# VivianDLi/CryoVIT

Hardware: AMD Instinct MI355X
Metric: tomogram voxels/sec (DINO feats + 3D seg fwd) (higher is better)
Workload: dtype bf16; 1 GPU; one 128x512x512 uint8 tomogram per step per GPU (configs[3]'s seeds 100..131, rank r takes 100 + r*steps + i): fused resize + DINOv2 ViT-g/14-reg (40 layers, N=1029 tokens/slice) -> fp16 dino_features [1536,128,32,32] + CryoVIT head [1,1536,128,32,32] -> probs [128,512,512] + masked Dice; synthetic weights; slice_batch=128, streams=1, parallelism=tomogram-sharded x1, no collectives

## Files before the change

cryovit_amd/check_asm.py:

```python

from __future__ import annotations

import re
import subprocess
import sys
import tempfile
from pathlib import Path

from cryovit_amd.build import ARCH, CSRC, FILE_FLAGS, FLAGS, INCLUDE, hipcc_path

EXPECTED_STORES = {"EpiSwiGLU": 8, "EpiBF16": 16, "EpiResidT": 32, "EpiResidHL": 33, "EpiVT": 16}


def compile_asm(src: Path) -> str:
    with tempfile.TemporaryDirectory() as td:
        out = Path(td) / (src.stem + ".s")
        flags = [f for f in FLAGS if f != "-fPIC"]
        cmd = [hipcc_path(), *flags, *FILE_FLAGS.get(src.name, []), "-I", str(INCLUDE), "-S", "--cuda-device-only", "-o", str(out), str(src)]
        r = subprocess.run(cmd, capture_output=True, text=True)
        if r.returncode != 0:
            raise RuntimeError(f"hipcc -S failed on {src.name}:\n{r.stderr}")
        return out.read_text()


def check_gemm256p(asm: str) -> list[str]:
    bodies = {m.group(1): m.group(2) for m in re.finditer(r"^(_ZN3cvx15k_gemm256p_[nm]reg\w+):.*?\n(.*?)s_endpgm", asm, re.S | re.M)}
    assert bodies, "no k_gemm256p kernels in the assembly"
    report = []
    for m in re.finditer(r"\.amdhsa_kernel (_ZN3cvx15k_gemm256p_[nm]reg\w+)(.*?)\.end_amdhsa_kernel", asm, re.S):
        name, desc = m.group(1), m.group(2)
        body = bodies[name]
        scratch = int(re.search(r"\.amdhsa_private_segment_fixed_size (\d+)", desc).group(1))
        vgpr = int(re.search(r"\.amdhsa_next_free_vgpr (\d+)", desc).group(1))
        assert scratch == 0 and "scratch_" not in body, f"{name}: spills to scratch ({scratch} B): uncounted vmcnt entries"
        assert vgpr <= 256, f"{name}: {vgpr} VGPRs"
        dma = re.findall(r"global_load_lds_dwordx4 (.*)", body)
        assert dma and all(re.fullmatch(r"v\d+, s\[\d+:\d+\]", d.strip()) for d in dma), f"{name}: LDS-DMA not in saddr form: {set(dma)}"
        stores = len(re.findall(r"global_store_", body))
        full = re.search(r"ELb1E(Lb[01]E)?EEv", name) is not None
        kind = next(k for k in EXPECTED_STORES if k in name)
        if full:
            assert stores == EXPECTED_STORES[kind], f"{name}: {stores} store instructions, the waits assume {EXPECTED_STORES[kind]}"
            assert all(s.startswith("global_store_dwordx4") for s in re.findall(r"global_store_\w+", body)), name
        report.append(f"{name[24:70]:48s} vgpr {vgpr:3d} stores {stores:2d} dma {len(dma):2d} {'FULL' if full else 'edge'}")
    return report


def check_dma_users(asm: str, fname: str) -> list[str]:
    report, inside, kernel, n_dma = [], False, None, {}
    for ln in asm.splitlines():
        t = ln.strip()
        m = re.match(r"^(_Z\w+):", ln)
        if m:
            kernel = m.group(1)
        if "#ASMSTART" in t:
            inside = True
        elif "#ASMEND" in t:
            inside = False
        elif t and not t.startswith((";", ".", "//")):
            if "global_load_lds" in t:
                n_dma[kernel] = n_dma.get(kernel, 0) + 1
            if not inside:
                assert "global_load_lds" not in t, f"{fname}:{kernel}: compiler-generated LDS-DMA: {t}"
                assert not re.search(r"\bm0\b", t), f"{fname}:{kernel}: M0 touched outside inline asm: {t}"
    for m in re.finditer(r"\.amdhsa_kernel (\w+)(.*?)\.end_amdhsa_kernel", asm, re.S):
        name, desc = m.group(1), m.group(2)
        if name not in n_dma:
            continue
        scratch = int(re.search(r"\.amdhsa_private_segment_fixed_size (\d+)", desc).group(1))
        vgpr = int(re.search(r"\.amdhsa_next_free_vgpr (\d+)", desc).group(1))
        assert scratch == 0, f"{fname}:{name}: {scratch} B of scratch in a kernel with counted vector-memory waits"
        report.append(f"{fname:16s} {name[:60]:60s} vgpr {vgpr:3d} dma {n_dma[name]:3d}")
    return report


DMA_SOURCES = ("attention.hip", "conv_halo.hip")


def main() -> None:
    gemm_asm = compile_asm(CSRC / "gemm.hip")
    for line in check_gemm256p(gemm_asm):
        print(line)
    for line in check_dma_users(gemm_asm, "gemm.hip"):
        print(line)
    for f in DMA_SOURCES:
        for line in check_dma_users(compile_asm(CSRC / f), f):
            print(line)
    print("ok")


if __name__ == "__main__":
    assert ARCH == "gfx950"
    main()
```

cryovit_amd/csrc/attention.hip:

```cpp
#include "common.h"
#include "../../include/cryovit_hip.h"
#include "host_util.h"
#include <atomic>
#include <string.h>

namespace cvx {

constexpr int ATT_THREADS = 256;
constexpr int KV_TILE = 64;
constexpr int ATT_TILE_BYTES = 64 * 128;
constexpr int ATT_XCD_REMAP = 1;
constexpr int ATT_PRIO_QK = 2;
constexpr int ATT_PRIO_PV = 4;
constexpr int ATT_FULL_LAST_TILE = 8;

__device__ __forceinline__ int pi_row(int r) { return (r & 0x13) | ((r & 4) << 1) | ((r & 8) >> 1); }

enum class Softmax { RunningMax, TileMax, ProbSum };
struct AttnCfg {
    int waves = 4;
    int nbuf = 2;
    Softmax softmax = Softmax::RunningMax;
    bool legacy = false;
    bool no_exp = false, no_sync = false, no_dma = false;
};
constexpr AttnCfg attn_cfg(int variant) {
    AttnCfg c;
    switch (variant) {
        case 1: c.legacy = true; break;
        case 3: c.nbuf = 3; break;
        case 6: c.softmax = Softmax::TileMax; break;
        case 7: c.softmax = Softmax::ProbSum; break;
        case 8: c.softmax = Softmax::ProbSum; c.waves = 8; c.nbuf = 3; break;
        case 9: c.softmax = Softmax::ProbSum; c.waves = 8; break;
        case 10: c.no_exp = true; break;
        case 11: c.no_sync = c.no_dma = true; break;
        case 12: c.no_sync = true; break;
        case 13: c.no_dma = true; break;
    }
    return c;
}

struct BlockCoord { int qb, slice, head; };
__device__ __forceinline__ BlockCoord block_coord(int flags, int nqb, int heads) {
    int qb, pair;
    if (flags & ATT_XCD_REMAP) {
        const int xcd = blockIdx.x & 7, w = blockIdx.x >> 3;
        pair = (w / nqb) * 8 + xcd;
        qb = w % nqb;
    } else {
        pair = blockIdx.x / nqb;
        qb = blockIdx.x % nqb;
    }
    return {qb, pair / heads, pair % heads};
}

__device__ __forceinline__ float row_max(const f32x16 (&s)[2]) {
    float m = s[0][0];
#pragma unroll
    for (int i = 1; i < 16; ++i) m = fmaxf(m, s[0][i]);
#pragma unroll
    for (int i = 0; i < 16; ++i) m = fmaxf(m, s[1][i]);
    return fmaxf(m, __shfl_xor(m, 32, 64));
}

__device__ __forceinline__ void exp2_sum(f32x16 (&s)[2], float& psum) {
    psum = 0.f;
#pragma unroll
    for (int t = 0; t < 2; ++t)
#pragma unroll
        for (int i = 0; i < 16; ++i) {
            const float p = __builtin_amdgcn_exp2f(s[t][i]);
            s[t][i] = p;
            psum += p;
        }
}

typedef short v4s_t __attribute__((ext_vector_type(4)));
typedef short v8s_t __attribute__((ext_vector_type(8)));
template <int VARIANT, bool VROW = false>
__global__ __launch_bounds__(attn_cfg(VARIANT).waves * 64) void k_attention(const uint16_t* __restrict__ qk, long ldqk,
                                                                            const uint16_t* __restrict__ vt, uint16_t* __restrict__ out,
                                                                            long ldo, int heads, int ntok, int ntp, int kp, int C, int nqb,
                                                                            int flags) {
    constexpr AttnCfg cfg = attn_cfg(VARIANT);
    constexpr int NW = cfg.waves, NBUF = cfg.nbuf;
    constexpr int NT = NW * 64, QB = NW * 32;
    constexpr int PPT = 512 / NT;
    constexpr bool AUG = cfg.softmax != Softmax::RunningMax, PSUM_TRIGGER = cfg.softmax == Softmax::ProbSum;
    constexpr bool LEGACY = cfg.legacy, ABL_NOEXP = cfg.no_exp, ABL_NOSYNC = cfg.no_sync, ABL_NODMA = cfg.no_dma;
    __shared__ __attribute__((aligned(16))) char smem[NBUF * 2 * ATT_TILE_BYTES];
    const int tid = threadIdx.x, lane = tid & 63;
    const int wave = __builtin_amdgcn_readfirstlane(tid >> 6);
    const bool prio_qk = (flags & ATT_PRIO_QK) != 0, prio_pv = (flags & ATT_PRIO_PV) != 0;
    const BlockCoord bc = block_coord(flags, nqb, heads);
    const int qb = bc.qb, slice = bc.slice, head = bc.head;
    const long row0 = (long)slice * ntp;
    const uint16_t* Qp = qk + row0 * ldqk + head * 64;
    const uint16_t* Kp = Qp + C;
    const uint16_t* Vp = VROW ? Kp + C : vt + ((long)(slice * heads + head) * 64) * kp;
    const long vpitch = VROW ? ldqk : (long)kp;

    const int r = lane & 31, h = lane >> 5;
    const int q0 = qb * QB + wave * 32;
    const int qrow = min(q0 + r, ntp - 1);
    const bool wave_idle = !LEGACY && q0 >= ntok;

    bf16x8 qf[4];
    {
        const uint16_t* qsrc = Qp + (long)qrow * ldqk + 8 * h;
#pragma unroll
        for (int ks = 0; ks < 4; ++ks) asm volatile("global_load_dwordx4 %0, %1, off" : "=v"(qf[ks]) : "v"(qsrc + 16 * ks) : "memory");
    }
    constexpr float DEFER = 3.0f;
    bf16x8 kaug, qaug;
    [[maybe_unused]] float m_used = 0.f;
    if constexpr (AUG) {
#pragma unroll
        for (int e = 0; e < 8; ++e) { kaug[e] = (__bf16)0.f; qaug[e] = (__bf16)0.f; }
        if (h == 0) kaug[0] = (__bf16)1.0f;
    }

    uint32_t koffs[2], voffs[2];
#pragma unroll
    for (int jj = 0; jj < 2; ++jj) {
        const int c = (jj < PPT ? jj : 0) * NT + tid;
        const int srow = c >> 3, schunk = ((c & 7) ^ ((srow >> 1) & 7)) << 3;
        koffs[jj] = (uint32_t)(srow * ldqk + schunk) * 2u;
        voffs[jj] = (uint32_t)(srow * vpitch + schunk) * 2u;
    }
    const bool lone = AUG && qb * QB + 32 >= ntok;
    if (lone && wave != 0) return;
    auto issue = [&](int j, int buf) {
        const uint32_t kt = lds_addr(smem) + buf * 2 * ATT_TILE_BYTES + wave * 1024;
        const long kv0 = (long)j * KV_TILE;
        if constexpr (PPT == 2) {
            glds16_saddr2<NT * 16>(Kp + kv0 * ldqk, koffs[0], koffs[1], kt);
            glds16_saddr2<NT * 16>(Vp + (VROW ? kv0 * ldqk : kv0), voffs[0], voffs[1], kt + ATT_TILE_BYTES);
        } else {
            glds16_saddr(Kp + kv0 * ldqk, koffs[0], kt);
            glds16_saddr(Vp + (VROW ? kv0 * ldqk : kv0), voffs[0], kt + ATT_TILE_BYTES);
        }
        if (lone) {
            uint32_t k0 = koffs[0], k1 = koffs[1], v0 = voffs[0], v1 = voffs[1];
            asm volatile("" : "+v"(k0), "+v"(k1), "+v"(v0), "+v"(v1));
#pragma unroll 1
            for (int w2 = 1; w2 < NW; ++w2) {
                const uint32_t fl = (w2 & 1) ? 64u : 0u;
                const uint32_t dk = (uint32_t)(w2 * 16) * (uint32_t)ldqk, dv = (uint32_t)(w2 * 16) * (uint32_t)vpitch;
                if constexpr (PPT == 2) {
                    glds16_saddr2<NT * 16>(Kp + kv0 * ldqk, (k0 + dk) ^ fl, (k1 + dk) ^ fl, kt + w2 * 1024);
                    glds16_saddr2<NT * 16>(Vp + (VROW ? kv0 * ldqk : kv0), (v0 + dv) ^ fl, (v1 + dv) ^ fl, kt + ATT_TILE_BYTES + w2 * 1024);
                } else {
                    glds16_saddr(Kp + kv0 * ldqk, (k0 + dk) ^ fl, kt + w2 * 1024);
                    glds16_saddr(Vp + (VROW ? kv0 * ldqk : kv0), (v0 + dv) ^ fl, kt + ATT_TILE_BYTES + w2 * 1024);
                }
            }
        }
    };

    const int krow = pi_row(r);
    const int koff = krow * 128, ksw = (krow >> 1) & 7;
    const int voff = r * 128, vsw = (r >> 1) & 7;
    [[maybe_unused]] uint32_t vtr[2][2];
    if constexpr (VROW) {
        const int li = lane & 15, dgrp = (lane >> 4) & 1;
#pragma unroll
        for (int dt = 0; dt < 2; ++dt)
#pragma unroll
            for (int j = 0; j < 2; ++j) {
                const int row = 8 * h + 4 * j + (li >> 2);
                const int chunk = (4 * dt + 2 * dgrp + ((li & 3) >> 1)) ^ ((row >> 1) & 7);
                vtr[dt][j] = (uint32_t)(row * 128 + (chunk << 4) + (li & 1) * 8);
            }
    }

    f32x16 o[2];
#pragma unroll
    for (int i = 0; i < 16; ++i) { o[0][i] = 0.f; o[1][i] = 0.f; }
    float m_run = -INFINITY, l_run = 0.f;

    const int nkv = (ntok + KV_TILE - 1) / KV_TILE;
    issue(0, 0);
    if (NBUF == 3 && nkv > 1) issue(1, 1);
    asm volatile("s_waitcnt vmcnt(0)" : "+v"(qf[0]), "+v"(qf[1]), "+v"(qf[2]), "+v"(qf[3])::"memory");
    int buf = 0;
    const char* kt = smem;
    [[maybe_unused]] bool redo = false;
    for (int j = 0; j < nkv; ++j) {
        if (!PSUM_TRIGGER || !redo) {
        if (!ABL_NOSYNC || j == 0) {
            if (NBUF == 3 && j + 1 < nkv) {
                if (lone) asm volatile("s_waitcnt vmcnt(%0)" ::"n"(2 * PPT * NW) : "memory");
                else asm volatile("s_waitcnt vmcnt(%0)" ::"n"(2 * PPT) : "memory");
            } else asm volatile("s_waitcnt vmcnt(0)" ::: "memory");
            __builtin_amdgcn_s_barrier();
        }
        if (NBUF == 3) {
            if (j + 2 < nkv) issue(j + 2, buf == 0 ? 2 : buf - 1);
        } else if (!ABL_NODMA && j + 1 < nkv) {
            issue(ABL_NOSYNC ? 0 : j + 1, ABL_NOSYNC ? 1 : (buf ^ 1));
        }
        kt = smem + (ABL_NOSYNC || ABL_NODMA ? 0 : buf) * 2 * ATT_TILE_BYTES;
        buf = NBUF == 3 ? (buf == 2 ? 0 : buf + 1) : (buf ^ 1);
        }
        [[maybe_unused]] const bool anchor = j == 0 || redo;
        redo = false;
        const char* vtile = kt + ATT_TILE_BYTES;
        if (wave_idle) continue;

        f32x16 s[2];
        const int kv0 = j * KV_TILE;
        const bool half_tile = !(flags & ATT_FULL_LAST_TILE) && kv0 + 32 >= ntok;
        auto compute_s = [&]() {
#pragma unroll
            for (int i = 0; i < 16; ++i) { s[0][i] = 0.f; s[1][i] = 0.f; }
            if (prio_qk) __builtin_amdgcn_s_setprio(1);
#pragma unroll
            for (int t = 0; t < 2; ++t) {
                if (t == 1 && half_tile) break;
                if constexpr (AUG) s[t] = __builtin_amdgcn_mfma_f32_32x32x16_bf16(kaug, qaug, s[t], 0, 0, 0);
#pragma unroll
                for (int ks = 0; ks < 4; ++ks) {
                    const bf16x8 kf = *(const bf16x8*)(kt + t * 4096 + koff + (((2 * ks + h) ^ ksw) << 4));
                    s[t] = __builtin_amdgcn_mfma_f32_32x32x16_bf16(kf, qf[ks], s[t], 0, 0, 0);
                }
            }
            if (prio_qk) __builtin_amdgcn_s_setprio(0);
            if (kv0 + KV_TILE > ntok) {
#pragma unroll
                for (int t = 0; t < 2; ++t)
#pragma unroll
                    for (int i = 0; i < 16; ++i) {
                        const int rho = (i & 3) + 8 * (i >> 2) + 4 * h;
                        if (kv0 + 32 * t + pi_row(rho) >= ntok) s[t][i] = -INFINITY;
                    }
            }
        };
        compute_s();

        if constexpr (PSUM_TRIGGER) {
            float psum;
            if (anchor) {
                const float mloc = row_max(s);
                const float m_new = (float)(__bf16)(m_used + (j == 0 ? mloc : fmaxf(mloc, 0.f)));
                const float delta = m_new - m_used;
                m_used = m_new;
                if (h == 0) qaug[0] = (__bf16)(-m_new);
                const float alpha = j == 0 ? 1.0f : __builtin_amdgcn_exp2f(-delta);
                l_run *= alpha;
#pragma unroll
                for (int i = 0; i < 16; ++i) { o[0][i] *= alpha; o[1][i] *= alpha; s[0][i] -= delta; s[1][i] -= delta; }
            }
            exp2_sum(s, psum);
            if (!anchor && __builtin_amdgcn_ballot_w64(!(psum <= 16777216.0f)) != 0) {
                redo = true;
                --j;
                continue;
            }
            l_run += psum;
        } else if constexpr (AUG) {
            const float mloc = row_max(s);
            if (j == 0 || __builtin_amdgcn_ballot_w64(mloc > DEFER) != 0) {
                const float m_new = (float)(__bf16)(m_used + (j == 0 ? mloc : fmaxf(mloc, 0.f)));
                const float delta = m_new - m_used;
                m_used = m_new;
                if (h == 0) qaug[0] = (__bf16)(-m_new);
                const float alpha = j == 0 ? 1.0f : __builtin_amdgcn_exp2f(-delta);
                l_run *= alpha;
#pragma unroll
                for (int i = 0; i < 16; ++i) { o[0][i] *= alpha; o[1][i] *= alpha; s[0][i] -= delta; s[1][i] -= delta; }
            }
            float psum;
            exp2_sum(s, psum);
            l_run += psum;
        } else {
            const float m_new = fmaxf(m_run, row_max(s));
            const float alpha = __builtin_amdgcn_exp2f(m_run - m_new);
            m_run = m_new;
            float psum = 0.f;
#pragma unroll
            for (int t = 0; t < 2; ++t)
#pragma unroll
                for (int i = 0; i < 16; ++i) {
                    const float p = ABL_NOEXP ? (s[t][i] - m_new) * 0.001f : __builtin_amdgcn_exp2f(s[t][i] - m_new);
                    s[t][i] = p;
                    psum += p;
                }
            l_run = fmaf(l_run, alpha, psum);
            if (LEGACY || __builtin_amdgcn_ballot_w64(alpha != 1.0f) != 0) {
#pragma unroll
                for (int i = 0; i < 16; ++i) { o[0][i] *= alpha; o[1][i] *= alpha; }
            }
        }

        if (prio_pv) __builtin_amdgcn_s_setprio(1);
#pragma unroll
        for (int t = 0; t < 2; ++t) {
            if (t == 1 && half_tile) break;
#pragma unroll
            for (int sk = 0; sk < 2; ++sk) {
                bf16x8 pf;
#pragma unroll
                for (int e = 0; e < 8; ++e) pf[e] = (__bf16)s[t][8 * sk + e];
#pragma unroll
                for (int dt = 0; dt < 2; ++dt) {
                    bf16x8 vf;
                    if constexpr (VROW) {
                        typedef __attribute__((address_space(3))) v4s_t* lds_v4;
                        const char* vb = vtile + (32 * t + 16 * sk) * 128;
                        const v4s_t a = __builtin_amdgcn_ds_read_tr16_b64_v4i16((lds_v4)(vb + vtr[dt][0]));
                        const v4s_t b = __builtin_amdgcn_ds_read_tr16_b64_v4i16((lds_v4)(vb + vtr[dt][1]));
                        vf = __builtin_bit_cast(bf16x8, v8s_t{a[0], a[1], a[2], a[3], b[0], b[1], b[2], b[3]});
                    } else {
                        vf = *(const bf16x8*)(vtile + dt * 4096 + voff + (((4 * t + 2 * sk + h) ^ vsw) << 4));
                    }
                    o[dt] = __builtin_amdgcn_mfma_f32_32x32x16_bf16(vf, pf, o[dt], 0, 0, 0);
                }
            }
        }
        if (prio_pv) __builtin_amdgcn_s_setprio(0);
    }

    const float l_tot = l_run + __shfl_xor(l_run, 32, 64);
    const float inv = 1.0f / l_tot;
    if (q0 + r < ntok) {
        uint16_t* orow = out + (row0 + q0 + r) * ldo + head * 64;
#pragma unroll
        for (int dt = 0; dt < 2; ++dt)
#pragma unroll
            for (int g = 0; g < 4; ++g) {
                uint2 w;
                w.x = pack2bf(o[dt][4 * g + 0] * inv, o[dt][4 * g + 1] * inv);
                w.y = pack2bf(o[dt][4 * g + 2] * inv, o[dt][4 * g + 3] * inv);
                *(uint2*)(orow + 32 * dt + 8 * g + 4 * h) = w;
            }
    }
}

#ifdef CVX_ABLATION
template <int NW>
__global__ __launch_bounds__(NW * 64) void k_attention64(const uint16_t* __restrict__ qk, long ldqk, const uint16_t* __restrict__ vt,
                                                         uint16_t* __restrict__ out, long ldo, int heads, int ntok, int ntp, int kp,
                                                         int C, int nqb, int flags) {
    constexpr int NT = NW * 64;
    __shared__ __attribute__((aligned(16))) char smem[2 * 2 * ATT_TILE_BYTES];
    const int tid = threadIdx.x, lane = tid & 63;
    const int wave = __builtin_amdgcn_readfirstlane(tid >> 6);
    const BlockCoord bc = block_coord(flags, nqb, heads);
    const int qb = bc.qb, slice = bc.slice, head = bc.head;
    const long row0 = (long)slice * ntp;
    const uint16_t* Qp = qk + row0 * ldqk + head * 64;
    const uint16_t* Kp = Qp + C;
    const uint16_t* Vp = vt + ((long)(slice * heads + head) * 64) * kp;
    const int r = lane & 31, h = lane >> 5;
    const int q0 = qb * NT + wave * 64;

    bf16x8 qf[2][4];
#pragma unroll
    for (int g = 0; g < 2; ++g) {
        const int qrow = min(q0 + 32 * g + r, ntp - 1);
#pragma unroll
        for (int ks = 0; ks < 4; ++ks) qf[g][ks] = *(const bf16x8*)(Qp + (long)qrow * ldqk + 16 * ks + 8 * h);
    }
    constexpr int NP = (512 + NT - 1) / NT;
    uint32_t koffs[NP], voffs[NP];
#pragma unroll
    for (int jj = 0; jj < NP; ++jj) {
        const int c = jj * NT + tid;
        const int srow = (c >> 3) & 63, schunk = ((c & 7) ^ ((srow >> 1) & 7)) << 3;
        koffs[jj] = (uint32_t)(srow * ldqk + schunk) * 2u;
        voffs[jj] = (uint32_t)(srow * kp + schunk) * 2u;
    }
    auto issue = [&](int j, int buf) {
        const uint32_t kt = lds_addr(smem) + buf * 2 * ATT_TILE_BYTES;
        const long kv0 = (long)j * KV_TILE;
#pragma unroll
        for (int jj = 0; jj < NP; ++jj) {
            if (jj * NT + wave * 64 >= 512) break;
            glds16_saddr(Kp + kv0 * ldqk, koffs[jj], kt + (jj * NT + wave * 64) * 16);
            glds16_saddr(Vp + kv0, voffs[jj], kt + ATT_TILE_BYTES + (jj * NT + wave * 64) * 16);
        }
    };
    const int krow = pi_row(r);
    const int koff = krow * 128, ksw = (krow >> 1) & 7;
    const int voff = r * 128, vsw = (r >> 1) & 7;

    f32x16 o[2][2];
#pragma unroll
    for (int g = 0; g < 2; ++g)
#pragma unroll
        for (int i = 0; i < 16; ++i) { o[g][0][i] = 0.f; o[g][1][i] = 0.f; }
    float m_run[2] = {-INFINITY, -INFINITY}, l_run[2] = {0.f, 0.f};
    const int nkv = (ntok + KV_TILE - 1) / KV_TILE;

    issue(0, 0);
    for (int j = 0; j < nkv; ++j) {
        asm volatile("s_waitcnt vmcnt(0)" ::: "memory");
        __syncthreads();
        if (j + 1 < nkv) issue(j + 1, (j + 1) & 1);
        const char* kt = smem + (j & 1) * 2 * ATT_TILE_BYTES;
        const char* vtile = kt + ATT_TILE_BYTES;

        f32x16 s[2][2];
#pragma unroll
        for (int g = 0; g < 2; ++g)
#pragma unroll
            for (int i = 0; i < 16; ++i) { s[g][0][i] = 0.f; s[g][1][i] = 0.f; }
#pragma unroll
        for (int t = 0; t < 2; ++t)
#pragma unroll
            for (int ks = 0; ks < 4; ++ks) {
                const bf16x8 kf = *(const bf16x8*)(kt + t * 4096 + koff + (((2 * ks + h) ^ ksw) << 4));
                s[0][t] = __builtin_amdgcn_mfma_f32_32x32x16_bf16(kf, qf[0][ks], s[0][t], 0, 0, 0);
                s[1][t] = __builtin_amdgcn_mfma_f32_32x32x16_bf16(kf, qf[1][ks], s[1][t], 0, 0, 0);
            }
        const int kv0 = j * KV_TILE;
        if (kv0 + KV_TILE > ntok) {
#pragma unroll
            for (int g = 0; g < 2; ++g)
#pragma unroll
                for (int t = 0; t < 2; ++t)
#pragma unroll
                    for (int i = 0; i < 16; ++i) {
                        const int rho = (i & 3) + 8 * (i >> 2) + 4 * h;
                        if (kv0 + 32 * t + pi_row(rho) >= ntok) s[g][t][i] = -INFINITY;
                    }
        }
#pragma unroll
        for (int g = 0; g < 2; ++g) {
            const float m_new = fmaxf(m_run[g], row_max(s[g]));
            const float alpha = __builtin_amdgcn_exp2f(m_run[g] - m_new);
            m_run[g] = m_new;
            float psum = 0.f;
#pragma unroll
            for (int t = 0; t < 2; ++t)
#pragma unroll
                for (int i = 0; i < 16; ++i) {
                    const float p = __builtin_amdgcn_exp2f(s[g][t][i] - m_new);
                    s[g][t][i] = p;
                    psum += p;
                }
            l_run[g] = fmaf(l_run[g], alpha, psum);
            if (__builtin_amdgcn_ballot_w64(alpha != 1.0f) != 0) {
#pragma unroll
                for (int i = 0; i < 16; ++i) { o[g][0][i] *= alpha; o[g][1][i] *= alpha; }
            }
        }
#pragma unroll
        for (int t = 0; t < 2; ++t)
#pragma unroll
            for (int sk = 0; sk < 2; ++sk) {
                bf16x8 pf[2];
#pragma unroll
                for (int g = 0; g < 2; ++g)
#pragma unroll
                    for (int e = 0; e < 8; ++e) pf[g][e] = (__bf16)s[g][t][8 * sk + e];
#pragma unroll
                for (int dt = 0; dt < 2; ++dt) {
                    const bf16x8 vf = *(const bf16x8*)(vtile + dt * 4096 + voff + (((4 * t + 2 * sk + h) ^ vsw) << 4));
                    o[0][dt] = __builtin_amdgcn_mfma_f32_32x32x16_bf16(vf, pf[0], o[0][dt], 0, 0, 0);
                    o[1][dt] = __builtin_amdgcn_mfma_f32_32x32x16_bf16(vf, pf[1], o[1][dt], 0, 0, 0);
                }
            }
    }
#pragma unroll
    for (int g = 0; g < 2; ++g) {
        const float l_tot = l_run[g] + __shfl_xor(l_run[g], 32, 64);
        const float inv = 1.0f / l_tot;
        const int q = q0 + 32 * g + r;
        if (q < ntok) {
            uint16_t* orow = out + (row0 + q) * ldo + head * 64;
#pragma unroll
            for (int dt = 0; dt < 2; ++dt)
#pragma unroll
                for (int gg = 0; gg < 4; ++gg) {
                    uint2 w;
                    w.x = pack2bf(o[g][dt][4 * gg + 0] * inv, o[g][dt][4 * gg + 1] * inv);
                    w.y = pack2bf(o[g][dt][4 * gg + 2] * inv, o[g][dt][4 * gg + 3] * inv);
                    *(uint2*)(orow + 32 * dt + 8 * gg + 4 * h) = w;
                }
        }
    }
}

#endif

}

using namespace cvx;

typedef void (*attn_kernel_t)(const uint16_t*, long, const uint16_t*, uint16_t*, long, int, int, int, int, int, int, int);
struct AttnVariant {
    int id;
    attn_kernel_t kernel;
    int threads, rows;
    bool needs_ld64;
};
template <int V>
static AttnVariant attn_row() {
    constexpr AttnCfg c = attn_cfg(V);
    return {V, k_attention<V, false>, c.waves * 64, c.waves * 32, c.softmax != Softmax::RunningMax};
}
static const AttnVariant g_attn_variants[] = {
    attn_row<0>(),
    attn_row<7>(),
#ifdef CVX_ABLATION
    attn_row<1>(), attn_row<3>(), attn_row<6>(),
    attn_row<8>(),
    attn_row<9>(),
    attn_row<10>(), attn_row<11>(), attn_row<12>(), attn_row<13>(),
    {4, k_attention64<3>, 192, 192, false},
    {5, k_attention64<4>, 256, 256, false},
#endif
};
static const AttnVariant* find_attn_variant(int id) {
    for (const AttnVariant& v : g_attn_variants)
        if (v.id == id) return &v;
    return nullptr;
}

static std::atomic<int> g_attn_variant{7};
static std::atomic<int> g_attn_xcd_remap{1};
static std::atomic<int> g_attn_half_tile{1};
static std::atomic<int> g_attn_mfma_prio{2};

int cvx_attn_set_option(const char* name, int value) {
    if (!strcmp(name, "attn_variant")) {
        if (!find_attn_variant(value)) return cvx_fail("set_option: unknown attn_variant (ablation variants need a -DCVX_ABLATION build)");
        g_attn_variant = value;
    } else if (!strcmp(name, "attn_xcd_remap")) g_attn_xcd_remap = value != 0;
    else if (!strcmp(name, "attn_mfma_prio")) g_attn_mfma_prio = value & 3;
    else if (!strcmp(name, "attn_half_tile")) g_attn_half_tile = value != 0;
    else return cvx_fail("set_option: unknown option");
    return 0;
}

static int attn_launch_flags(long pairs) {
    const int prio = g_attn_mfma_prio;
    return (pairs % 8 == 0 && g_attn_xcd_remap ? ATT_XCD_REMAP : 0) | (prio & 1 ? ATT_PRIO_QK : 0) | (prio & 2 ? ATT_PRIO_PV : 0) |
           (g_attn_half_tile ? 0 : ATT_FULL_LAST_TILE);
}

static int launch_attention(const AttnVariant& v, const char* grid_msg, const void* qk, long ldqk, const void* vt, void* out, long ldo,
                            int slices, int heads, int ntok, int ntp, int kp, hipStream_t st) {
    const int nqb = (ntok + v.rows - 1) / v.rows;
    const long nblk = (long)nqb * heads * slices;
    if (nblk > 0x7fffffff) return cvx_fail(grid_msg);
    hipLaunchKernelGGL(v.kernel, dim3((unsigned)nblk), dim3(v.threads), 0, st, (const uint16_t*)qk, ldqk, (const uint16_t*)vt, (uint16_t*)out,
                       ldo, heads, ntok, ntp, kp, heads * 64, nqb, attn_launch_flags((long)heads * slices));
    return cvx_check_launch();
}

extern "C" int cvx_attention_qkv_bf16(const void* qkv, long ld, void* out, long ldo, int slices, int heads, int ntok, int ntp,
                                      hipStream_t st) {
    if (slices <= 0) return 0;
    if (!qkv || !out) return cvx_fail("attention_qkv: null pointer");
    if (ntp % 8 || ntp < ntok || ld % 64 || ld < 3L * heads * 64 || ldo % 4)
        return cvx_fail("attention_qkv: need ntp%8==0, ntp>=ntok, ld%64==0 (the default kernel's lone-wave DMA offsets), ld >= 3*heads*64");
    const AttnVariant v = {7, k_attention<7, true>, ATT_THREADS, 128, true};
    return launch_attention(v, "attention_qkv: grid too large", qkv, ld, nullptr, out, ldo, slices, heads, ntok, ntp,  0, st);
}

extern "C" int cvx_attention_bf16(const void* qk, long ldqk, const void* vt, void* out, long ldo, int slices, int heads,
                                  int ntok, int ntp, int kp, hipStream_t st) {
    if (slices <= 0) return 0;
    if (ntp % 8 || kp % 64 || kp < ntok || ntp < ntok || ldqk % 8 || ldo % 4)
        return cvx_fail("attention: need ntp%8==0, kp%64==0, kp>=ntok, ntp>=ntok, ldqk%8==0");
    const AttnVariant* v = find_attn_variant(g_attn_variant);
    if (v->needs_ld64 && ldqk % 64 != 0) v = find_attn_variant(0);
    return launch_attention(*v, "attention: grid too large", qk, ldqk, vt, out, ldo, slices, heads, ntok, ntp, kp, st);
}
```

Measured before the change: 116.0 million voxels/s.

## Generalize attention kernel to two query groups per wave and specialize default flags

Rewrites the attention kernel so each wave can process one or two 32-row query groups sharing every K/V LDS fragment read, with per-group ProbSum softmax state and a redo path for groups whose sums overflow. The old separate k_attention64 variants become configs 4/5 of the unified kernel. Adds a compile-time specialization (DEF) for the default flag set, so the common launch drops the runtime priority and full-last-tile checks. The qkv entry point now follows the selected variant. The default stays variant 7 with one group, so the main change on the default path is the specialized kernel and the restructured loop. The asm checker gains a test that no compiler-placed vmcnt waits sit inside the key loop.

```diff
diff --git a/cryovit_amd/check_asm.py b/cryovit_amd/check_asm.py
--- a/cryovit_amd/check_asm.py
+++ b/cryovit_amd/check_asm.py
@@ -12,11 +12,11 @@
 EXPECTED_STORES = {"EpiSwiGLU": 8, "EpiBF16": 16, "EpiResidT": 32, "EpiResidHL": 33, "EpiVT": 16}
 
 
-def compile_asm(src: Path) -> str:
+def compile_asm(src: Path, defines: tuple[str, ...] = ()) -> str:
     with tempfile.TemporaryDirectory() as td:
         out = Path(td) / (src.stem + ".s")
         flags = [f for f in FLAGS if f != "-fPIC"]
-        cmd = [hipcc_path(), *flags, *FILE_FLAGS.get(src.name, []), "-I", str(INCLUDE), "-S", "--cuda-device-only", "-o", str(out), str(src)]
+        cmd = [hipcc_path(), *flags, *defines, *FILE_FLAGS.get(src.name, []), "-I", str(INCLUDE), "-S", "--cuda-device-only", "-o", str(out), str(src)]
         r = subprocess.run(cmd, capture_output=True, text=True)
         if r.returncode != 0:
             raise RuntimeError(f"hipcc -S failed on {src.name}:\n{r.stderr}")
@@ -74,6 +74,36 @@
     return report
 
 
+def check_attention_loop_waits(asm: str) -> list[str]:
+    report = []
+    descs = {m.group(1): m.group(2) for m in re.finditer(r"\.amdhsa_kernel (\w+)(.*?)\.end_amdhsa_kernel", asm, re.S)}
+    for m in re.finditer(r"^(_ZN3cvx11k_attentionILi([457])E\w+):.*?\n(.*?)s_endpgm", asm, re.S | re.M):
+        name, variant, body = m.group(1), int(m.group(2)), m.group(3).splitlines()
+        scratch = int(re.search(r"\.amdhsa_private_segment_fixed_size (\d+)", descs[name]).group(1))
+        vgpr = int(re.search(r"\.amdhsa_next_free_vgpr (\d+)", descs[name]).group(1))
+        assert scratch == 0, f"{name}: {scratch} B of scratch"
+        assert vgpr <= (128 if variant == 7 else 256), f"{name}: {vgpr} VGPRs"
+        labels = {mm.group(1): i for i, ln in enumerate(body) if (mm := re.match(r"^(\.LBB\d+_\d+):", ln))}
+        barriers = [i for i, ln in enumerate(body) if re.search(r"\bs_barrier\b", ln)]
+        assert len(barriers) == 1, f"{name}: {len(barriers)} barriers, expected the key loop's one"
+        bar = barriers[0]
+        back = [i for i, ln in enumerate(body) for t in re.findall(r"\bs_c?branch\w* (\.LBB\d+_\d+)", ln) if labels.get(t, len(body)) < bar < i]
+        assert back, f"{name}: no backward branch round the barrier"
+        inside, written, total = False, 0, 0
+        for ln in body[bar : max(back) + 1]:
+            if "#ASMSTART" in ln:
+                inside = True
+            elif "#ASMEND" in ln:
+                inside = False
+            elif re.search(r"\bs_waitcnt\b.*\bvmcnt", ln):
+                total += 1
+                written += inside
+        assert total == written, f"{name}: {total - written} compiler-placed vmcnt waits inside the key loop (they drain the tile prefetch)"
+        report.append(f"{name[:60]:60s} vgpr {vgpr:3d} loop lines {max(back) - bar:4d} vmcnt waits in loop {total} (written {written})")
+    assert report, "no ProbSum attention kernels in the assembly"
+    return report
+
+
 DMA_SOURCES = ("attention.hip", "conv_halo.hip")
 
 
@@ -86,6 +116,8 @@
     for f in DMA_SOURCES:
         for line in check_dma_users(compile_asm(CSRC / f), f):
             print(line)
+    for line in check_attention_loop_waits(compile_asm(CSRC / "attention.hip", defines=("-DCVX_ABLATION",))):
+        print(line)
     print("ok")
 
 
diff --git a/cryovit_amd/csrc/attention.hip b/cryovit_amd/csrc/attention.hip
--- a/cryovit_amd/csrc/attention.hip
+++ b/cryovit_amd/csrc/attention.hip
@@ -6,7 +6,6 @@
 
 namespace cvx {
 
-constexpr int ATT_THREADS = 256;
 constexpr int KV_TILE = 64;
 constexpr int ATT_TILE_BYTES = 64 * 128;
 constexpr int ATT_XCD_REMAP = 1;
@@ -19,6 +18,7 @@
 enum class Softmax { RunningMax, TileMax, ProbSum };
 struct AttnCfg {
     int waves = 4;
+    int groups = 1;
     int nbuf = 2;
     Softmax softmax = Softmax::RunningMax;
     bool legacy = false;
@@ -29,6 +29,8 @@
     switch (variant) {
         case 1: c.legacy = true; break;
         case 3: c.nbuf = 3; break;
+        case 4: c.softmax = Softmax::ProbSum; c.groups = 2; c.waves = 2; break;
+        case 5: c.softmax = Softmax::ProbSum; c.groups = 2; break;
         case 6: c.softmax = Softmax::TileMax; break;
         case 7: c.softmax = Softmax::ProbSum; break;
         case 8: c.softmax = Softmax::ProbSum; c.waves = 8; c.nbuf = 3; break;
@@ -78,21 +80,24 @@
 
 typedef short v4s_t __attribute__((ext_vector_type(4)));
 typedef short v8s_t __attribute__((ext_vector_type(8)));
-template <int VARIANT, bool VROW = false>
-__global__ __launch_bounds__(attn_cfg(VARIANT).waves * 64) void k_attention(const uint16_t* __restrict__ qk, long ldqk,
+template <int I> struct IntC { static constexpr int value = I; };
+template <int VARIANT, bool VROW = false, bool DEF = false>
+__global__ __launch_bounds__(attn_cfg(VARIANT).waves * 64) __attribute__((amdgpu_waves_per_eu(attn_cfg(VARIANT).groups))) void k_attention(const uint16_t* __restrict__ qk, long ldqk,
                                                                             const uint16_t* __restrict__ vt, uint16_t* __restrict__ out,
                                                                             long ldo, int heads, int ntok, int ntp, int kp, int C, int nqb,
                                                                             int flags) {
     constexpr AttnCfg cfg = attn_cfg(VARIANT);
-    constexpr int NW = cfg.waves, NBUF = cfg.nbuf;
-    constexpr int NT = NW * 64, QB = NW * 32;
+    constexpr int NW = cfg.waves, NBUF = cfg.nbuf, G = cfg.groups;
+    constexpr int NT = NW * 64, RPW = 32 * G, QB = NW * RPW;
     constexpr int PPT = 512 / NT;
     constexpr bool AUG = cfg.softmax != Softmax::RunningMax, PSUM_TRIGGER = cfg.softmax == Softmax::ProbSum;
     constexpr bool LEGACY = cfg.legacy, ABL_NOEXP = cfg.no_exp, ABL_NOSYNC = cfg.no_sync, ABL_NODMA = cfg.no_dma;
+    static_assert(G == 1 || (G == 2 && PSUM_TRIGGER && NBUF == 2), "two groups per wave: ProbSum softmax, two buffers");
     __shared__ __attribute__((aligned(16))) char smem[NBUF * 2 * ATT_TILE_BYTES];
     const int tid = threadIdx.x, lane = tid & 63;
     const int wave = __builtin_amdgcn_readfirstlane(tid >> 6);
-    const bool prio_qk = (flags & ATT_PRIO_QK) != 0, prio_pv = (flags & ATT_PRIO_PV) != 0;
+    const bool prio_qk = !DEF && (flags & ATT_PRIO_QK) != 0, prio_pv = DEF || (flags & ATT_PRIO_PV) != 0;
+    const bool full_last = !DEF && (flags & ATT_FULL_LAST_TILE) != 0;
     const BlockCoord bc = block_coord(flags, nqb, heads);
     const int qb = bc.qb, slice = bc.slice, head = bc.head;
     const long row0 = (long)slice * ntp;
@@ -102,23 +107,29 @@
     const long vpitch = VROW ? ldqk : (long)kp;
 
     const int r = lane & 31, h = lane >> 5;
-    const int q0 = qb * QB + wave * 32;
-    const int qrow = min(q0 + r, ntp - 1);
+    const int q0 = qb * QB + wave * RPW;
     const bool wave_idle = !LEGACY && q0 >= ntok;
-
-    bf16x8 qf[4];
-    {
-        const uint16_t* qsrc = Qp + (long)qrow * ldqk + 8 * h;
-#pragma unroll
-        for (int ks = 0; ks < 4; ++ks) asm volatile("global_load_dwordx4 %0, %1, off" : "=v"(qf[ks]) : "v"(qsrc + 16 * ks) : "memory");
+    const int alive = G == 2 && q0 + 32 < ntok ? 3 : 1;
+
+    bf16x8 qf[G][4];
+#pragma unroll
+    for (int g = 0; g < G; ++g) {
+        const uint16_t* qsrc = Qp + (long)min(q0 + 32 * g + r, ntp - 1) * ldqk + 8 * h;
+#pragma unroll
+        for (int ks = 0; ks < 4; ++ks) asm volatile("global_load_dwordx4 %0, %1, off" : "=v"(qf[g][ks]) : "v"(qsrc + 16 * ks) : "memory");
     }
     constexpr float DEFER = 3.0f;
-    bf16x8 kaug, qaug;
-    [[maybe_unused]] float m_used = 0.f;
+    bf16x8 kaug, qaug[G];
+    [[maybe_unused]] float m_used[G];
+#pragma unroll
+    for (int g = 0; g < G; ++g) m_used[g] = 0.f;
     if constexpr (AUG) {
 #pragma unroll
-        for (int e = 0; e < 8; ++e) { kaug[e] = (__bf16)0.f; qaug[e] = (__bf16)0.f; }
-        if (h == 0) kaug[0] = (__bf16)1.0f;
+        for (int e = 0; e < 8; ++e) {
+            kaug[e] = (__bf16)1.0f;
+#pragma unroll
+            for (int g = 0; g < G; ++g) qaug[g][e] = (__bf16)0.f;
+        }
     }
 
     uint32_t koffs[2], voffs[2];
@@ -129,18 +140,26 @@
         koffs[jj] = (uint32_t)(srow * ldqk + schunk) * 2u;
         voffs[jj] = (uint32_t)(srow * vpitch + schunk) * 2u;
     }
-    const bool lone = AUG && qb * QB + 32 >= ntok;
+    auto pieces = [&](const uint16_t* kb, const uint16_t* vb, uint32_t k0, uint32_t k1, uint32_t v0, uint32_t v1, uint32_t dst) {
+        if constexpr (PPT >= 2) {
+#pragma unroll
+            for (int p = 0; p < PPT / 2; ++p) {
+                glds16_saddr2<NT * 16>(kb + (long)p * (NT / 4) * ldqk, k0, k1, dst + p * 2 * NT * 16);
+                glds16_saddr2<NT * 16>(vb + (long)p * (NT / 4) * vpitch, v0, v1, dst + ATT_TILE_BYTES + p * 2 * NT * 16);
+            }
+        } else {
+            glds16_saddr(kb, k0, dst);
+            glds16_saddr(vb, v0, dst + ATT_TILE_BYTES);
+        }
+    };
+    const bool lone = AUG && qb * QB + RPW >= ntok;
     if (lone && wave != 0) return;
     auto issue = [&](int j, int buf) {
         const uint32_t kt = lds_addr(smem) + buf * 2 * ATT_TILE_BYTES + wave * 1024;
         const long kv0 = (long)j * KV_TILE;
-        if constexpr (PPT == 2) {
-            glds16_saddr2<NT * 16>(Kp + kv0 * ldqk, koffs[0], koffs[1], kt);
-            glds16_saddr2<NT * 16>(Vp + (VROW ? kv0 * ldqk : kv0), voffs[0], voffs[1], kt + ATT_TILE_BYTES);
-        } else {
-            glds16_saddr(Kp + kv0 * ldqk, koffs[0], kt);
-            glds16_saddr(Vp + (VROW ? kv0 * ldqk : kv0), voffs[0], kt + ATT_TILE_BYTES);
-        }
+        const uint16_t* kb = Kp + kv0 * ldqk;
+        const uint16_t* vb = Vp + (VROW ? kv0 * ldqk : kv0);
+        pieces(kb, vb, koffs[0], koffs[1], voffs[0], voffs[1], kt);
         if (lone) {
             uint32_t k0 = koffs[0], k1 = koffs[1], v0 = voffs[0], v1 = voffs[1];
             asm volatile("" : "+v"(k0), "+v"(k1), "+v"(v0), "+v"(v1));
@@ -148,13 +167,7 @@
             for (int w2 = 1; w2 < NW; ++w2) {
                 const uint32_t fl = (w2 & 1) ? 64u : 0u;
                 const uint32_t dk = (uint32_t)(w2 * 16) * (uint32_t)ldqk, dv = (uint32_t)(w2 * 16) * (uint32_t)vpitch;
-                if constexpr (PPT == 2) {
-                    glds16_saddr2<NT * 16>(Kp + kv0 * ldqk, (k0 + dk) ^ fl, (k1 + dk) ^ fl, kt + w2 * 1024);
-                    glds16_saddr2<NT * 16>(Vp + (VROW ? kv0 * ldqk : kv0), (v0 + dv) ^ fl, (v1 + dv) ^ fl, kt + ATT_TILE_BYTES + w2 * 1024);
-                } else {
-                    glds16_saddr(Kp + kv0 * ldqk, (k0 + dk) ^ fl, kt + w2 * 1024);
-                    glds16_saddr(Vp + (VROW ? kv0 * ldqk : kv0), (v0 + dv) ^ fl, kt + ATT_TILE_BYTES + w2 * 1024);
-                }
+                pieces(kb, vb, (k0 + dk) ^ fl, (k1 + dk) ^ fl, (v0 + dv) ^ fl, (v1 + dv) ^ fl, kt + w2 * 1024);
             }
         }
     };
@@ -175,19 +188,159 @@
             }
     }
 
-    f32x16 o[2];
-#pragma unroll
-    for (int i = 0; i < 16; ++i) { o[0][i] = 0.f; o[1][i] = 0.f; }
-    float m_run = -INFINITY, l_run = 0.f;
+    f32x16 o[G][2];
+    float m_run[G], l_run[G];
+#pragma unroll
+    for (int g = 0; g < G; ++g) {
+#pragma unroll
+        for (int i = 0; i < 16; ++i) { o[g][0][i] = 0.f; o[g][1][i] = 0.f; }
+        m_run[g] = -INFINITY;
+        l_run[g] = 0.f;
+    }
 
     const int nkv = (ntok + KV_TILE - 1) / KV_TILE;
+    const char* kt = smem;
+    int j = 0;
+
+    auto tile = [&](auto G0, auto G1, const int anchor) -> int {
+        constexpr int g0 = decltype(G0)::value, g1 = decltype(G1)::value;
+        const char* vtile = kt + ATT_TILE_BYTES;
+        const int kv0 = j * KV_TILE;
+        const bool half_tile = !full_last && kv0 + 32 >= ntok;
+        f32x16 s[G][2];
+        constexpr f32x16 zero = {};
+        if (prio_qk) __builtin_amdgcn_s_setprio(1);
+#pragma unroll
+        for (int t = 0; t < 2; ++t) {
+            if (t == 1 && half_tile) {
+#pragma unroll
+                for (int g = g0; g < g1; ++g)
+#pragma unroll
+                    for (int i = 0; i < 16; ++i) s[g][1][i] = 0.f;
+                break;
+            }
+            if constexpr (AUG) {
+#pragma unroll
+                for (int g = g0; g < g1; ++g) s[g][t] = __builtin_amdgcn_mfma_f32_32x32x16_bf16(kaug, qaug[g], zero, 0, 0, 0);
+            }
+#pragma unroll
+            for (int ks = 0; ks < 4; ++ks) {
+                const bf16x8 kf = *(const bf16x8*)(kt + t * 4096 + koff + (((2 * ks + h) ^ ksw) << 4));
+#pragma unroll
+                for (int g = g0; g < g1; ++g)
+                    s[g][t] = __builtin_amdgcn_mfma_f32_32x32x16_bf16(kf, qf[g][ks], AUG || ks > 0 ? s[g][t] : zero, 0, 0, 0);
+            }
+        }
+        if (prio_qk) __builtin_amdgcn_s_setprio(0);
+        if (kv0 + KV_TILE > ntok) {
+#pragma unroll
+            for (int g = g0; g < g1; ++g)
+#pragma unroll
+                for (int t = 0; t < 2; ++t)
+#pragma unroll
+                    for (int i = 0; i < 16; ++i) {
+                        const int rho = (i & 3) + 8 * (i >> 2) + 4 * h;
+                        if (kv0 + 32 * t + pi_row(rho) >= ntok) s[g][t][i] = -INFINITY;
+                    }
+        }
+
+        auto read_v = [&](int t, int sk, int dt) -> bf16x8 {
+            if constexpr (VROW) {
+                typedef __attribute__((address_space(3))) v4s_t* lds_v4;
+                const char* vb = vtile + (32 * t + 16 * sk) * 128;
+                const v4s_t a = __builtin_amdgcn_ds_read_tr16_b64_v4i16((lds_v4)(vb + vtr[dt][0]));
+                const v4s_t b = __builtin_amdgcn_ds_read_tr16_b64_v4i16((lds_v4)(vb + vtr[dt][1]));
+                return __builtin_bit_cast(bf16x8, v8s_t{a[0], a[1], a[2], a[3], b[0], b[1], b[2], b[3]});
+            } else {
+                return *(const bf16x8*)(vtile + dt * 4096 + voff + (((4 * t + 2 * sk + h) ^ vsw) << 4));
+            }
+        };
+        int again = 0;
+#pragma unroll
+        for (int g = g0; g < g1; ++g) {
+            if constexpr (PSUM_TRIGGER) {
+                float psum;
+                const bool anch = (anchor >> g) & 1;
+                if (anch) {
+                    const float mloc = row_max(s[g]);
+                    const float m_new = (float)(__bf16)(m_used[g] + (j == 0 ? mloc : fmaxf(mloc, 0.f)));
+                    const float delta = m_new - m_used[g];
+                    m_used[g] = m_new;
+                    if (h == 0) qaug[g][0] = (__bf16)(-m_new);
+                    const float alpha = j == 0 ? 1.0f : __builtin_amdgcn_exp2f(-delta);
+                    l_run[g] *= alpha;
+#pragma unroll
+                    for (int i = 0; i < 16; ++i) { o[g][0][i] *= alpha; o[g][1][i] *= alpha; s[g][0][i] -= delta; s[g][1][i] -= delta; }
+                }
+                exp2_sum(s[g], psum);
+                if (!anch && __builtin_amdgcn_ballot_w64(!(psum <= 16777216.0f)) != 0) {
+                    again |= 1 << g;
+                    continue;
+                }
+                l_run[g] += psum;
+            } else if constexpr (AUG) {
+                const float mloc = row_max(s[g]);
+                if (j == 0 || __builtin_amdgcn_ballot_w64(mloc > DEFER) != 0) {
+                    const float m_new = (float)(__bf16)(m_used[g] + (j == 0 ? mloc : fmaxf(mloc, 0.f)));
+                    const float delta = m_new - m_used[g];
+                    m_used[g] = m_new;
+                    if (h == 0) qaug[g][0] = (__bf16)(-m_new);
+                    const float alpha = j == 0 ? 1.0f : __builtin_amdgcn_exp2f(-delta);
+                    l_run[g] *= alpha;
+#pragma unroll
+                    for (int i = 0; i < 16; ++i) { o[g][0][i] *= alpha; o[g][1][i] *= alpha; s[g][0][i] -= delta; s[g][1][i] -= delta; }
+                }
+                float psum;
+                exp2_sum(s[g], psum);
+                l_run[g] += psum;
+            } else {
+                const float m_new = fmaxf(m_run[g], row_max(s[g]));
+                const float alpha = __builtin_amdgcn_exp2f(m_run[g] - m_new);
+                m_run[g] = m_new;
+                float psum = 0.f;
+#pragma unroll
+                for (int t = 0; t < 2; ++t)
+#pragma unroll
+                    for (int i = 0; i < 16; ++i) {
+                        const float p = ABL_NOEXP ? (s[g][t][i] - m_new) * 0.001f : __builtin_amdgcn_exp2f(s[g][t][i] - m_new);
+                        s[g][t][i] = p;
+                        psum += p;
+                    }
+                l_run[g] = fmaf(l_run[g], alpha, psum);
+                if (LEGACY || __builtin_amdgcn_ballot_w64(alpha != 1.0f) != 0) {
+#pragma unroll
+                    for (int i = 0; i < 16; ++i) { o[g][0][i] *= alpha; o[g][1][i] *= alpha; }
+                }
+            }
+
+            if (prio_pv) __builtin_amdgcn_s_setprio(1);
+#pragma unroll
+            for (int t = 0; t < 2; ++t) {
+                if (t == 1 && half_tile) break;
+#pragma unroll
+                for (int sk = 0; sk < 2; ++sk) {
+                    bf16x8 pf;
+#pragma unroll
+                    for (int e = 0; e < 8; ++e) pf[e] = (__bf16)s[g][t][8 * sk + e];
+#pragma unroll
+                    for (int dt = 0; dt < 2; ++dt) {
+                        const bf16x8 vf = read_v(t, sk, dt);
+                        o[g][dt] = __builtin_amdgcn_mfma_f32_32x32x16_bf16(vf, pf, o[g][dt], 0, 0, 0);
+                    }
+                }
+            }
+            if (prio_pv) __builtin_amdgcn_s_setprio(0);
+        }
+        return again;
+    };
+
     issue(0, 0);
     if (NBUF == 3 && nkv > 1) issue(1, 1);
-    asm volatile("s_waitcnt vmcnt(0)" : "+v"(qf[0]), "+v"(qf[1]), "+v"(qf[2]), "+v"(qf[3])::"memory");
+    asm volatile("s_waitcnt vmcnt(0)" : "+v"(qf[0][0]), "+v"(qf[0][1]), "+v"(qf[0][2]), "+v"(qf[0][3])::"memory");
+    if constexpr (G == 2) asm volatile("" : "+v"(qf[G - 1][0]), "+v"(qf[G - 1][1]), "+v"(qf[G - 1][2]), "+v"(qf[G - 1][3])::"memory");
     int buf = 0;
-    const char* kt = smem;
-    [[maybe_unused]] bool redo = false;
-    for (int j = 0; j < nkv; ++j) {
+    [[maybe_unused]] int redo = 0;
+    for (; j < nkv; ++j) {
         if (!PSUM_TRIGGER || !redo) {
         if (!ABL_NOSYNC || j == 0) {
             if (NBUF == 3 && j + 1 < nkv) {
@@ -204,273 +357,21 @@
         kt = smem + (ABL_NOSYNC || ABL_NODMA ? 0 : buf) * 2 * ATT_TILE_BYTES;
         buf = NBUF == 3 ? (buf == 2 ? 0 : buf + 1) : (buf ^ 1);
         }
-        [[maybe_unused]] const bool anchor = j == 0 || redo;
-        redo = false;
-        const char* vtile = kt + ATT_TILE_BYTES;
         if (wave_idle) continue;
-
-        f32x16 s[2];
-        const int kv0 = j * KV_TILE;
-        const bool half_tile = !(flags & ATT_FULL_LAST_TILE) && kv0 + 32 >= ntok;
-        auto compute_s = [&]() {
-#pragma unroll
-            for (int i = 0; i < 16; ++i) { s[0][i] = 0.f; s[1][i] = 0.f; }
-            if (prio_qk) __builtin_amdgcn_s_setprio(1);
-#pragma unroll
-            for (int t = 0; t < 2; ++t) {
-                if (t == 1 && half_tile) break;
-                if constexpr (AUG) s[t] = __builtin_amdgcn_mfma_f32_32x32x16_bf16(kaug, qaug, s[t], 0, 0, 0);
-#pragma unroll
-                for (int ks = 0; ks < 4; ++ks) {
-                    const bf16x8 kf = *(const bf16x8*)(kt + t * 4096 + koff + (((2 * ks + h) ^ ksw) << 4));
-                    s[t] = __builtin_amdgcn_mfma_f32_32x32x16_bf16(kf, qf[ks], s[t], 0, 0, 0);
-                }
-            }
-            if (prio_qk) __builtin_amdgcn_s_setprio(0);
-            if (kv0 + KV_TILE > ntok) {
-#pragma unroll
-                for (int t = 0; t < 2; ++t)
-#pragma unroll
-                    for (int i = 0; i < 16; ++i) {
-                        const int rho = (i & 3) + 8 * (i >> 2) + 4 * h;
-                        if (kv0 + 32 * t + pi_row(rho) >= ntok) s[t][i] = -INFINITY;
-                    }
-            }
-        };
-        compute_s();
-
-        if constexpr (PSUM_TRIGGER) {
-            float psum;
-            if (anchor) {
-                const float mloc = row_max(s);
-                const float m_new = (float)(__bf16)(m_used + (j == 0 ? mloc : fmaxf(mloc, 0.f)));
-                const float delta = m_new - m_used;
-                m_used = m_new;
-                if (h == 0) qaug[0] = (__bf16)(-m_new);
-                const float alpha = j == 0 ? 1.0f : __builtin_amdgcn_exp2f(-delta);
-                l_run *= alpha;
-#pragma unroll
-                for (int i = 0; i < 16; ++i) { o[0][i] *= alpha; o[1][i] *= alpha; s[0][i] -= delta; s[1][i] -= delta; }
-            }
-            exp2_sum(s, psum);
-            if (!anchor && __builtin_amdgcn_ballot_w64(!(psum <= 16777216.0f)) != 0) {
-                redo = true;
-                --j;
-                continue;
-            }
-            l_run += psum;
-        } else if constexpr (AUG) {
-            const float mloc = row_max(s);
-            if (j == 0 || __builtin_amdgcn_ballot_w64(mloc > DEFER) != 0) {
-                const float m_new = (float)(__bf16)(m_used + (j == 0 ? mloc : fmaxf(mloc, 0.f)));
-                const float delta = m_new - m_used;
-                m_used = m_new;
-                if (h == 0) qaug[0] = (__bf16)(-m_new);
-                const float alpha = j == 0 ? 1.0f : __builtin_amdgcn_exp2f(-delta);
-                l_run *= alpha;
-#pragma unroll
-                for (int i = 0; i < 16; ++i) { o[0][i] *= alpha; o[1][i] *= alpha; s[0][i] -= delta; s[1][i] -= delta; }
-            }
-            float psum;
-            exp2_sum(s, psum);
-            l_run += psum;
-        } else {
-            const float m_new = fmaxf(m_run, row_max(s));
-            const float alpha = __builtin_amdgcn_exp2f(m_run - m_new);
-            m_run = m_new;
-            float psum = 0.f;
-#pragma unroll
-            for (int t = 0; t < 2; ++t)
-#pragma unroll
-                for (int i = 0; i < 16; ++i) {
-                    const float p = ABL_NOEXP ? (s[t][i] - m_new) * 0.001f : __builtin_amdgcn_exp2f(s[t][i] - m_new);
-                    s[t][i] = p;
-                    psum += p;
-                }
-            l_run = fmaf(l_run, alpha, psum);
-            if (LEGACY || __builtin_amdgcn_ballot_w64(alpha != 1.0f) != 0) {
-#pragma unroll
-                for (int i = 0; i < 16; ++i) { o[0][i] *= alpha; o[1][i] *= alpha; }
-            }
-        }
-
-        if (prio_pv) __builtin_amdgcn_s_setprio(1);
-#pragma unroll
-        for (int t = 0; t < 2; ++t) {
-            if (t == 1 && half_tile) break;
-#pragma unroll
-            for (int sk = 0; sk < 2; ++sk) {
-                bf16x8 pf;
-#pragma unroll
-                for (int e = 0; e < 8; ++e) pf[e] = (__bf16)s[t][8 * sk + e];
-#pragma unroll
-                for (int dt = 0; dt < 2; ++dt) {
-                    bf16x8 vf;
-                    if constexpr (VROW) {
-                        typedef __attribute__((address_space(3))) v4s_t* lds_v4;
-                        const char* vb = vtile + (32 * t + 16 * sk) * 128;
-                        const v4s_t a = __builtin_amdgcn_ds_read_tr16_b64_v4i16((lds_v4)(vb + vtr[dt][0]));
-                        const v4s_t b = __builtin_amdgcn_ds_read_tr16_b64_v4i16((lds_v4)(vb + vtr[dt][1]));
-                        vf = __builtin_bit_cast(bf16x8, v8s_t{a[0], a[1], a[2], a[3], b[0], b[1], b[2], b[3]});
-                    } else {
-                        vf = *(const bf16x8*)(vtile + dt * 4096 + voff + (((4 * t + 2 * sk + h) ^ vsw) << 4));
-                    }
-                    o[dt] = __builtin_amdgcn_mfma_f32_32x32x16_bf16(vf, pf, o[dt], 0, 0, 0);
-                }
-            }
-        }
-        if (prio_pv) __builtin_amdgcn_s_setprio(0);
-    }
-
-    const float l_tot = l_run + __shfl_xor(l_run, 32, 64);
-    const float inv = 1.0f / l_tot;
-    if (q0 + r < ntok) {
-        uint16_t* orow = out + (row0 + q0 + r) * ldo + head * 64;
-#pragma unroll
-        for (int dt = 0; dt < 2; ++dt)
-#pragma unroll
-            for (int g = 0; g < 4; ++g) {
-                uint2 w;
-                w.x = pack2bf(o[dt][4 * g + 0] * inv, o[dt][4 * g + 1] * inv);
-                w.y = pack2bf(o[dt][4 * g + 2] * inv, o[dt][4 * g + 3] * inv);
-                *(uint2*)(orow + 32 * dt + 8 * g + 4 * h) = w;
-            }
-    }
-}
-
-#ifdef CVX_ABLATION
-template <int NW>
-__global__ __launch_bounds__(NW * 64) void k_attention64(const uint16_t* __restrict__ qk, long ldqk, const uint16_t* __restrict__ vt,
-                                                         uint16_t* __restrict__ out, long ldo, int heads, int ntok, int ntp, int kp,
-                                                         int C, int nqb, int flags) {
-    constexpr int NT = NW * 64;
-    __shared__ __attribute__((aligned(16))) char smem[2 * 2 * ATT_TILE_BYTES];
-    const int tid = threadIdx.x, lane = tid & 63;
-    const int wave = __builtin_amdgcn_readfirstlane(tid >> 6);
-    const BlockCoord bc = block_coord(flags, nqb, heads);
-    const int qb = bc.qb, slice = bc.slice, head = bc.head;
-    const long row0 = (long)slice * ntp;
-    const uint16_t* Qp = qk + row0 * ldqk + head * 64;
-    const uint16_t* Kp = Qp + C;
-    const uint16_t* Vp = vt + ((long)(slice * heads + head) * 64) * kp;
-    const int r = lane & 31, h = lane >> 5;
-    const int q0 = qb * NT + wave * 64;
-
-    bf16x8 qf[2][4];
-#pragma unroll
-    for (int g = 0; g < 2; ++g) {
-        const int qrow = min(q0 + 32 * g + r, ntp - 1);
-#pragma unroll
-        for (int ks = 0; ks < 4; ++ks) qf[g][ks] = *(const bf16x8*)(Qp + (long)qrow * ldqk + 16 * ks + 8 * h);
-    }
-    constexpr int NP = (512 + NT - 1) / NT;
-    uint32_t koffs[NP], voffs[NP];
-#pragma unroll
-    for (int jj = 0; jj < NP; ++jj) {
-        const int c = jj * NT + tid;
-        const int srow = (c >> 3) & 63, schunk = ((c & 7) ^ ((srow >> 1) & 7)) << 3;
-        koffs[jj] = (uint32_t)(srow * ldqk + schunk) * 2u;
-        voffs[jj] = (uint32_t)(srow * kp + schunk) * 2u;
-    }
-    auto issue = [&](int j, int buf) {
-        const uint32_t kt = lds_addr(smem) + buf * 2 * ATT_TILE_BYTES;
-        const long kv0 = (long)j * KV_TILE;
-#pragma unroll
-        for (int jj = 0; jj < NP; ++jj) {
-            if (jj * NT + wave * 64 >= 512) break;
-            glds16_saddr(Kp + kv0 * ldqk, koffs[jj], kt + (jj * NT + wave * 64) * 16);
-            glds16_saddr(Vp + kv0, voffs[jj], kt + ATT_TILE_BYTES + (jj * NT + wave * 64) * 16);
-        }
-    };
-    const int krow = pi_row(r);
-    const int koff = krow * 128, ksw = (krow >> 1) & 7;
-    const int voff = r * 128, vsw = (r >> 1) & 7;
-
-    f32x16 o[2][2];
-#pragma unroll
-    for (int g = 0; g < 2; ++g)
-#pragma unroll
-        for (int i = 0; i < 16; ++i) { o[g][0][i] = 0.f; o[g][1][i] = 0.f; }
-    float m_run[2] = {-INFINITY, -INFINITY}, l_run[2] = {0.f, 0.f};
-    const int nkv = (ntok + KV_TILE - 1) / KV_TILE;
-
-    issue(0, 0);
-    for (int j = 0; j < nkv; ++j) {
-        asm volatile("s_waitcnt vmcnt(0)" ::: "memory");
-        __syncthreads();
-        if (j + 1 < nkv) issue(j + 1, (j + 1) & 1);
-        const char* kt = smem + (j & 1) * 2 * ATT_TILE_BYTES;
-        const char* vtile = kt + ATT_TILE_BYTES;
-
-        f32x16 s[2][2];
-#pragma unroll
-        for (int g = 0; g < 2; ++g)
-#pragma unroll
-            for (int i = 0; i < 16; ++i) { s[g][0][i] = 0.f; s[g][1][i] = 0.f; }
-#pragma unroll
-        for (int t = 0; t < 2; ++t)
-#pragma unroll
-            for (int ks = 0; ks < 4; ++ks) {
-                const bf16x8 kf = *(const bf16x8*)(kt + t * 4096 + koff + (((2 * ks + h) ^ ksw) << 4));
-                s[0][t] = __builtin_amdgcn_mfma_f32_32x32x16_bf16(kf, qf[0][ks], s[0][t], 0, 0, 0);
-                s[1][t] = __builtin_amdgcn_mfma_f32_32x32x16_bf16(kf, qf[1][ks], s[1][t], 0, 0, 0);
-            }
-        const int kv0 = j * KV_TILE;
-        if (kv0 + KV_TILE > ntok) {
-#pragma unroll
-            for (int g = 0; g < 2; ++g)
-#pragma unroll
-                for (int t = 0; t < 2; ++t)
-#pragma unroll
-                    for (int i = 0; i < 16; ++i) {
-                        const int rho = (i & 3) + 8 * (i >> 2) + 4 * h;
-                        if (kv0 + 32 * t + pi_row(rho) >= ntok) s[g][t][i] = -INFINITY;
-                    }
-        }
-#pragma unroll
-        for (int g = 0; g < 2; ++g) {
-            const float m_new = fmaxf(m_run[g], row_max(s[g]));
-            const float alpha = __builtin_amdgcn_exp2f(m_run[g] - m_new);
-            m_run[g] = m_new;
-            float psum = 0.f;
-#pragma unroll
-            for (int t = 0; t < 2; ++t)
-#pragma unroll
-                for (int i = 0; i < 16; ++i) {
-                    const float p = __builtin_amdgcn_exp2f(s[g][t][i] - m_new);
-                    s[g][t][i] = p;
-                    psum += p;
-                }
-            l_run[g] = fmaf(l_run[g], alpha, psum);
-            if (__builtin_amdgcn_ballot_w64(alpha != 1.0f) != 0) {
-#pragma unroll
-                for (int i = 0; i < 16; ++i) { o[g][0][i] *= alpha; o[g][1][i] *= alpha; }
-            }
-        }
-#pragma unroll
-        for (int t = 0; t < 2; ++t)
-#pragma unroll
-            for (int sk = 0; sk < 2; ++sk) {
-                bf16x8 pf[2];
-#pragma unroll
-                for (int g = 0; g < 2; ++g)
-#pragma unroll
-                    for (int e = 0; e < 8; ++e) pf[g][e] = (__bf16)s[g][t][8 * sk + e];
-#pragma unroll
-                for (int dt = 0; dt < 2; ++dt) {
-                    const bf16x8 vf = *(const bf16x8*)(vtile + dt * 4096 + voff + (((4 * t + 2 * sk + h) ^ vsw) << 4));
-                    o[0][dt] = __builtin_amdgcn_mfma_f32_32x32x16_bf16(vf, pf[0], o[0][dt], 0, 0, 0);
-                    o[1][dt] = __builtin_amdgcn_mfma_f32_32x32x16_bf16(vf, pf[1], o[1][dt], 0, 0, 0);
-                }
-            }
-    }
-#pragma unroll
-    for (int g = 0; g < 2; ++g) {
+        const int anchor = j == 0 ? 3 : redo;
+        const int act = redo ? redo : alive;
+        if (G == 1 || act == 3) redo = tile(IntC<0>(), IntC<G>(), anchor);
+        else if (act == 1) redo = tile(IntC<0>(), IntC<1>(), anchor);
+        else redo = tile(IntC<G - 1>(), IntC<G>(), anchor);
+        if (redo) --j;
+    }
+
+#pragma unroll
+    for (int g = 0; g < G; ++g) {
         const float l_tot = l_run[g] + __shfl_xor(l_run[g], 32, 64);
         const float inv = 1.0f / l_tot;
-        const int q = q0 + 32 * g + r;
-        if (q < ntok) {
-            uint16_t* orow = out + (row0 + q) * ldo + head * 64;
+        if (q0 + 32 * g + r < ntok) {
+            uint16_t* orow = out + (row0 + q0 + 32 * g + r) * ldo + head * 64;
 #pragma unroll
             for (int dt = 0; dt < 2; ++dt)
 #pragma unroll
@@ -484,8 +385,6 @@
     }
 }
 
-#endif
-
 }
 
 using namespace cvx;
@@ -493,25 +392,34 @@
 typedef void (*attn_kernel_t)(const uint16_t*, long, const uint16_t*, uint16_t*, long, int, int, int, int, int, int, int);
 struct AttnVariant {
     int id;
-    attn_kernel_t kernel;
+    attn_kernel_t kernel[2], kernel_def[2];
     int threads, rows;
     bool needs_ld64;
 };
+constexpr int ATT_DEFAULT_VARIANT = 7;
 template <int V>
 static AttnVariant attn_row() {
     constexpr AttnCfg c = attn_cfg(V);
-    return {V, k_attention<V, false>, c.waves * 64, c.waves * 32, c.softmax != Softmax::RunningMax};
+    return {V, {k_attention<V, false>, nullptr}, {nullptr, nullptr}, c.waves * 64, c.waves * c.groups * 32, c.softmax != Softmax::RunningMax};
+}
+template <int V>
+static AttnVariant attn_row_full() {
+    AttnVariant v = attn_row<V>();
+    v.kernel[1] = k_attention<V, true>;
+    v.kernel_def[0] = k_attention<V, false, true>;
+    v.kernel_def[1] = k_attention<V, true, true>;
+    return v;
 }
 static const AttnVariant g_attn_variants[] = {
     attn_row<0>(),
-    attn_row<7>(),
+    attn_row_full<7>(),
 #ifdef CVX_ABLATION
     attn_row<1>(), attn_row<3>(), attn_row<6>(),
     attn_row<8>(),
     attn_row<9>(),
     attn_row<10>(), attn_row<11>(), attn_row<12>(), attn_row<13>(),
-    {4, k_attention64<3>, 192, 192, false},
-    {5, k_attention64<4>, 256, 256, false},
+    attn_row_full<4>(),
+    attn_row_full<5>(),
 #endif
 };
 static const AttnVariant* find_attn_variant(int id) {
@@ -520,7 +428,7 @@
     return nullptr;
 }
 
-static std::atomic<int> g_attn_variant{7};
+static std::atomic<int> g_attn_variant{ATT_DEFAULT_VARIANT};
 static std::atomic<int> g_attn_xcd_remap{1};
 static std::atomic<int> g_attn_half_tile{1};
 static std::atomic<int> g_attn_mfma_prio{2};
@@ -542,13 +450,15 @@
            (g_attn_half_tile ? 0 : ATT_FULL_LAST_TILE);
 }
 
-static int launch_attention(const AttnVariant& v, const char* grid_msg, const void* qk, long ldqk, const void* vt, void* out, long ldo,
+static int launch_attention(const AttnVariant& v, int vrow, const char* grid_msg, const void* qk, long ldqk, const void* vt, void* out, long ldo,
                             int slices, int heads, int ntok, int ntp, int kp, hipStream_t st) {
     const int nqb = (ntok + v.rows - 1) / v.rows;
     const long nblk = (long)nqb * heads * slices;
     if (nblk > 0x7fffffff) return cvx_fail(grid_msg);
-    hipLaunchKernelGGL(v.kernel, dim3((unsigned)nblk), dim3(v.threads), 0, st, (const uint16_t*)qk, ldqk, (const uint16_t*)vt, (uint16_t*)out,
-                       ldo, heads, ntok, ntp, kp, heads * 64, nqb, attn_launch_flags((long)heads * slices));
+    const int flags = attn_launch_flags((long)heads * slices);
+    const bool def = (flags & ~ATT_XCD_REMAP) == ATT_PRIO_PV && v.kernel_def[vrow];
+    hipLaunchKernelGGL(def ? v.kernel_def[vrow] : v.kernel[vrow], dim3((unsigned)nblk), dim3(v.threads), 0, st, (const uint16_t*)qk, ldqk,
+                       (const uint16_t*)vt, (uint16_t*)out, ldo, heads, ntok, ntp, kp, heads * 64, nqb, flags);
     return cvx_check_launch();
 }
 
@@ -558,8 +468,9 @@
     if (!qkv || !out) return cvx_fail("attention_qkv: null pointer");
     if (ntp % 8 || ntp < ntok || ld % 64 || ld < 3L * heads * 64 || ldo % 4)
         return cvx_fail("attention_qkv: need ntp%8==0, ntp>=ntok, ld%64==0 (the default kernel's lone-wave DMA offsets), ld >= 3*heads*64");
-    const AttnVariant v = {7, k_attention<7, true>, ATT_THREADS, 128, true};
-    return launch_attention(v, "attention_qkv: grid too large", qkv, ld, nullptr, out, ldo, slices, heads, ntok, ntp,  0, st);
+    const AttnVariant* v = find_attn_variant(g_attn_variant);
+    if (!v->kernel[1]) v = find_attn_variant(ATT_DEFAULT_VARIANT);
+    return launch_attention(*v, 1, "attention_qkv: grid too large", qkv, ld, nullptr, out, ldo, slices, heads, ntok, ntp,  0, st);
 }
 
 extern "C" int cvx_attention_bf16(const void* qk, long ldqk, const void* vt, void* out, long ldo, int slices, int heads,
@@ -569,5 +480,5 @@
         return cvx_fail("attention: need ntp%8==0, kp%64==0, kp>=ntok, ntp>=ntok, ldqk%8==0");
     const AttnVariant* v = find_attn_variant(g_attn_variant);
     if (v->needs_ld64 && ldqk % 64 != 0) v = find_attn_variant(0);
-    return launch_attention(*v, "attention: grid too large", qk, ldqk, vt, out, ldo, slices, heads, ntok, ntp, kp, st);
-}
+    return launch_attention(*v, 0, "attention: grid too large", qk, ldqk, vt, out, ldo, slices, heads, ntok, ntp, kp, st);
+}
```

New measurement: 116.0 million voxels/s. About the same (-0.0%).
